# alessiomelone/Ternary-spGEMM

Measured on AMD Instinct MI355X. Metric: effective GFLOP/s + achieved HBM GB/s (% roofline), TCSC spGEMM M×K×N at s, higher is better.
Workload: dtype f32

## Files before the change

ternary-spgemm_amd/csrc/tsg_capi.cpp:

```cpp
#include <hip/hip_runtime.h>

#include <algorithm>
#include <cmath>
#include <cstdlib>
#include <cstdio>
#include <cstring>
#include <atomic>
#include <iterator>
#include <condition_variable>
#include <mutex>
#include <string>
#include <thread>
#include <vector>

#include "../../include/ternary_spgemm_test.h"
#include "tsg_internal.h"
#include "tsg_plan.h"

using tsg::CallPlan;
using tsg::JitShape;
using tsg::Kernel;

extern thread_local std::string g_tsg_host_err;

// ... 61 lines not shown
namespace {

struct DeviceGuard {
    int prev = -1;
    explicit DeviceGuard(int dev)
    {
        if (hipGetDevice(&prev) != hipSuccess) prev = -1;
        if (dev >= 0 && dev != prev) (void)hipSetDevice(dev);
    }
    ~DeviceGuard()
    {
        if (prev >= 0) (void)hipSetDevice(prev);
    }
};

int check_device(int dev)
{
    hipDeviceProp_t prop;
    if (hipGetDeviceProperties(&prop, dev) != hipSuccess)
        return fail(TSG_ERR_NODEV, "hipGetDeviceProperties failed for device " + std::to_string(dev));
    if (std::strncmp(prop.gcnArchName, "gfx950", 6) != 0)
        return fail(TSG_ERR_NODEV, std::string("device is ") + prop.gcnArchName +
                                       "; this library is built for gfx950 (MI355X) only");
    return TSG_OK;
}

struct XtDims {
    int Mp, Kp;
};
XtDims dims_for(int M, int K, int tile_m, int chunk)
{
    return {((std::max(M, 1) + tile_m - 1) / tile_m) * tile_m, std::max(1, (K + chunk - 1) / chunk) * chunk};
}

int ensure_work(tsg_tcsc *h, int M, int tile_m, int chunk, bool capturing)
{
    const XtDims d = dims_for(M, h->plan.K, tile_m, chunk);
    const size_t need = (size_t)d.Mp * d.Kp * sizeof(float);
// ... 295 lines not shown
    if (!direct) {
        rc = work_begin(h, p, c);
        if (rc) return rc;
        if (K == 0) {
            HIP_TRY(hipMemsetAsync(h->d_work, 0, (size_t)d.Mp * d.Kp * sizeof(float), c.s));
        } else if ((r64 ? tsg::launch_transpose_quads(c.dX, h->d_work, c.M, K, d.Mp, d.Kp, jv.piece_rows, c.s, p.chunk)
                        : tsg::launch_transpose_pairs(c.dX, h->d_work, c.M, K, d.Mp, d.Kp, c.s)) != 0) {
            return fail(TSG_ERR_HIP, std::string("transpose launch: ") + hipGetErrorString(hipGetLastError()));
        }
    }
    int slot;
    rc = timing_begin(h, c.capturing, c.s, slot);
    if (rc) return rc;
    if (tsg::launch_tcsc_jit(jv.mod, direct ? c.dX : h->d_work, d.Mp, jv.d_wcode, c.db, c.dalpha, c.dY, c.M, N, jv.Npad,
                             jv.nch, c.prelu ? 1 : 0, h->d_status, jv.nw * jv.waves, waves, p.gn, p.gm, p.tmask, c.s,
                             p.tile_m, direct ? K : 0, lastadj, p.xtouch, p.tnear) != 0)
        return fail(TSG_ERR_HIP, std::string("tcsc launch: ") + hipGetErrorString(hipGetLastError()));
    rc = timing_end(h, slot, c.s);
    if (rc || direct) return rc;
    return work_end(h, c);
}

int run_dev(tsg_tcsc *h, const float *dX, const float *db, const float *dalpha, float *dY, int M,
            int N, int K, hipStream_t s, bool prelu)
{
    if (!h) return fail(TSG_ERR_ARG, "null handle");
    if (N != h->plan.N || K != h->plan.K)
        return fail(TSG_ERR_ARG, "shape mismatch: handle has K=" + std::to_string(h->plan.K) + " N=" +
                                     std::to_string(h->plan.N) + ", call has K=" + std::to_string(K) +
                                     " N=" + std::to_string(N));
    if (M < 0) return fail(TSG_ERR_ARG, "M < 0");
// ... 219 lines not shown
{
    if (!out) return fail(TSG_ERR_ARG, "null out");
    *out = nullptr;
    if (B < 0) return fail(TSG_ERR_ARG, "negative block size");
    const std::string ke = tsg::knob_check();
    if (!ke.empty()) return fail(TSG_ERR_ARG, ke);
    std::string e = tsg::validate_tcsc(csp, csn, rip, rin, K, N, B);
    if (!e.empty()) return fail(TSG_ERR_ARG, std::string(B ? "malformed BlockedTCSC: " : "malformed TCSC: ") + e);
    if (B && (tsg::kJitXRegs - tsg::kJitNW) / tsg::kJitSlotRegs < 2)
        return fail(TSG_ERR_ARG, "BlockedTCSC: this jit kernel geometry has no registers for the block sums");
    const int64_t slots = (B ? (int64_t)(K / B) : 1) * N;
    int ndev = 0;
    if (hipGetDeviceCount(&ndev) != hipSuccess || ndev == 0) return fail(TSG_ERR_NODEV, "no HIP device");
    if (device < 0) HIP_TRY(hipGetDevice(&device));
    if (device >= ndev) return fail(TSG_ERR_ARG, "device index out of range");
    int rc = check_device(device);
    if (rc) return rc;

    tsg_tcsc *h = new tsg_tcsc();
    h->plan.K = K;
    h->plan.N = N;
    h->plan.B = B;
    h->device = device;
    {
        DeviceGuard g0(device);
        if (hipStreamCreateWithFlags(&h->stream, hipStreamNonBlocking) != hipSuccess) {
            delete h;
            return fail(TSG_ERR_HIP, "hipStreamCreate of the handle's stream failed");
        }
    }
    h->nnz_pos = csp[slots];
    h->nnz_neg = csn[slots];
    h->plan.nnz = h->nnz_pos + h->nnz_neg;
    h->csp.assign(csp, csp + slots + 1);
// ... 336 lines not shown
    *gn = p.gn;
    *gm = p.gm;
    *tmask = p.tmask;
    return TSG_OK;
}

extern "C" int tsg_call_xtouch(int K, int N, int64_t nnz, int M)
{
    if (K < 0 || N <= 0 || nnz < 0 || nnz > (int64_t)K * N || M <= 0) {
        g_tsg_host_err = "tsg_call_xtouch: bad arguments";
        return TSG_ERR_ARG;
    }
    return tsg::plan_call(plain_input(K, N, nnz), M).xtouch;
}

extern "C" const char *tcsc_hip_call_kernel(const tsg_tcsc *h, int M)
{
    if (!h) return "";
    std::lock_guard<std::mutex> lk(h->mu);
    switch (tsg::plan_call(h->plan, M).kernel) {
    case Kernel::kEllPc: return "tsg_tcsc_ell_pc_kernel";
    case Kernel::kEll: return "tsg_tcsc_ell_kernel";
    case Kernel::kJit64: return "tsg_jit64_kernel";
    case Kernel::kJit128: return "tsg_jit_kernel";
    case Kernel::kRx: break;
    }
    return "tsg_tcsc_rx_kernel";
}

extern "C" int64_t tcsc_hip_call_image_bytes(tsg_tcsc *h, int M)
// ... 107 lines not shown
```

ternary-spgemm_amd/csrc/tsg_internal.h:

```cpp
#pragma once

#include <cstddef>
#include <cstdint>
#include <string>
#include <vector>

namespace tsg {

constexpr int kLanes = 64;

#ifndef TSG_RX_WAVES
#define TSG_RX_WAVES 8
#endif
#ifndef TSG_RX_CHUNK
#define TSG_RX_CHUNK 64
#endif
#ifndef TSG_RX_ROWS
#define TSG_RX_ROWS 24
#endif
constexpr int kRxTileM = 256;
constexpr int kRxWaves = TSG_RX_WAVES;
constexpr int kRxNW = 32;
constexpr int kRxTileCols = kRxWaves * kRxNW;
constexpr int kRxChunk = TSG_RX_CHUNK;
// ... 68 lines not shown
                    const int32_t *rin, int K, int N, int B, JitImage &img, int nw = kJitNW,
                    int waves = kJitWaves, bool far = false, bool rows64 = false, bool half = false);

struct JitModule {
    void *module = nullptr;
    void *function = nullptr;
    void *probe = nullptr;
    std::string load(const std::vector<uint32_t> &code, int nw = kJitNW, int waves = kJitWaves,
                     bool rows64 = false, bool half = false, bool pair = false);
    void unload();
};
int launch_tcsc_jit(const JitModule &jm, const float *XT, int Mp, const uint32_t *wcode,
                    const float *b, const float *alpha, float *Y, int M, int N, int Npad, int nch,
                    int prelu, uint32_t *status, int tile_cols, int waves, int gn, int gm, int tmask,
                    void *stream, int tile_m = kJitTileM, int xrow = 0, int lastadj = 0, int xtouch = 0,
                    int tnear = 0);
int launch_jit_probe(const JitModule &jm, uint32_t *status, void *stream);

constexpr int kEllVariants = 5;
constexpr int kEllTileM[kEllVariants] = {1, 4, 8, 16, 32};
constexpr int kEllMaxC[kEllVariants] = {40956, 10236, 5116, 2556, 1276};
struct EllImage {
    int C = 0, nch = 0, steps = 0, nslices = 0;
    int xb = 0;
    int zr = 1;
    std::vector<uint32_t> ent;
    std::vector<uint32_t> tab;
};
constexpr int ell_copy_offset(int C, int MT) { return ((C + 1) * MT + 63) / 64 * 64 + 32; }
__host__ __device__ constexpr int ell_lds_floats(int C, int MT, int xb, int zr = 1)
{
// ... 35 lines not shown
```

ternary-spgemm_amd/csrc/tsg_jit.cpp:

```cpp
#include <hip/hip_runtime.h>

#include <dlfcn.h>
#include <elf.h>

#include <algorithm>
#include <cmath>
#include <cstdio>
#include <cstdlib>
#include <cstring>
#include <fstream>
#include <iterator>

#include "tsg_internal.h"
#include "tsg_jit_map.h"
#include "../../include/ternary_spgemm_test.h"

namespace tsg {

namespace {

struct Emit {
    std::vector<uint32_t> &c;
    bool pad8 = true;
    void align8()
// ... 788 lines not shown
    function = nullptr;
    probe = nullptr;
}

int launch_jit_probe(const JitModule &jm, uint32_t *status, void *stream)
{
    void *params[] = {(void *)&status};
    const hipError_t e =
        hipModuleLaunchKernel((hipFunction_t)jm.probe, 1, 1, 1, 64, 1, 1, 0, (hipStream_t)stream, params, nullptr);
    return e == hipSuccess ? 0 : -1;
}

int launch_tcsc_jit(const JitModule &jm, const float *XT, int Mp, const uint32_t *wcode, const float *b,
                    const float *alpha, float *Y, int M, int N, int Npad, int nch, int prelu,
                    uint32_t *status, int tile_cols, int waves, int gn, int gm, int tmask, void *stream,
                    int tile_m, int xrow, int lastadj, int xtouch, int tnear)
{
    int mtiles = Mp / tile_m, ntiles = Npad / tile_cols;
    void *params[] = {(void *)&XT, (void *)&Mp, (void *)&wcode, (void *)&b, (void *)&alpha, (void *)&Y,
                      (void *)&M, (void *)&N, (void *)&nch, (void *)&mtiles, (void *)&ntiles, (void *)&prelu,
                      (void *)&status, (void *)&gn, (void *)&gm, (void *)&tmask, (void *)&xrow, (void *)&lastadj,
                      (void *)&xtouch, (void *)&tnear};
    hipError_t e = hipModuleLaunchKernel((hipFunction_t)jm.function, (unsigned)(mtiles * ntiles), 1, 1,
                                         (unsigned)waves * 64u, 1, 1, 0, (hipStream_t)stream, params, nullptr);
    return e == hipSuccess ? 0 : -1;
}

}

extern thread_local std::string g_tsg_host_err;

extern "C" int tsg_jit_codegen_wv(const int32_t *csp, const int32_t *csn, const int32_t *rip, const int32_t *rin,
                                  int K, int N, int B, int width, int waves, uint32_t *code, int64_t code_cap,
                                  int64_t *code_len, uint32_t *wcode, int64_t wcode_cap, int64_t *wcode_len)
{
    if (!tsg::jit_waves_ok(width, waves)) {
        g_tsg_host_err = "tsg_jit_codegen: unsupported waves per workgroup " + std::to_string(waves) +
                         " for width " + std::to_string(width) + " (8; 4 for widths 32, 16, 8)";
// ... 158 lines not shown
```

ternary-spgemm_amd/csrc/tsg_jit_kernel.hip:

```cpp
#include <hip/hip_runtime.h>

#include <cstdint>

#include "tsg_jit_map.h"

namespace {

#ifndef TSG_JIT_NW
#define TSG_JIT_NW 64
#endif
#ifndef TSG_JIT_WAVES
#define TSG_JIT_WAVES 8
#endif
#ifndef TSG_JIT_ROWS64
#define TSG_JIT_ROWS64 0
#endif
#ifndef TSG_JIT_HALF
#define TSG_JIT_HALF 0
#endif
#ifndef TSG_JIT_PAIR
#define TSG_JIT_PAIR 0
#endif
constexpr int kJWaves = TSG_JIT_WAVES;
constexpr int kJNW = TSG_JIT_NW;
constexpr bool kJRows64 = TSG_JIT_ROWS64 != 0;
constexpr bool kJHalf = TSG_JIT_HALF != 0;
constexpr bool kJPair = TSG_JIT_PAIR != 0;
static_assert(!kJHalf || (kJRows64 && TSG_JIT_WAVES == 4), "the half ring is a 4-wave 64-row image");
static_assert(!kJPair || (kJRows64 && TSG_JIT_WAVES == 4 && !kJHalf), "wave pairs run the 4-wave 64-row image");
static_assert(kJNW == 64 || kJNW == 32 || kJNW == 16 || kJNW == 8 || (kJRows64 && kJNW == 128), "stream width");
static_assert(kJWaves == 8 || (kJWaves == 4 && kJNW < 64), "waves per workgroup");
constexpr int kJTileM = kJRows64 ? 64 : 128;
constexpr int kJRowsPerLane = kJTileM / 64;
constexpr int kJTileCols = kJWaves * kJNW;
constexpr int kJThreads = (kJPair ? 2 : 1) * kJWaves * 64;
constexpr int kJRing = 3;
constexpr int kJChunk = kJRows64 ? (kJHalf ? 96 : 192) : 96;
// ... 76 lines not shown

    uint64_t base;
    asm volatile("s_getpc_b64 s[92:93]\n\t"
                 "s_add_u32 s92, s92, 0x7a5e1234\n\t"
                 "s_addc_u32 s93, s93, 0"
                 : "={s[92:93]}"(base)
                 :
                 : "scc");
    const uint32_t *hdr = reinterpret_cast<const uint32_t *>(base);
    if (hdr[0] != kJMagic0 || hdr[1] != kJMagic1 || ((hdr[7] >> 8) & 0xffu) != kJFormat ||
        ((hdr[7] & kJHalfFlag) != 0) != kJHalf) {
        if (blockIdx.x == 0 && tid == 0) status[0] = 1u;
        return;
    }

    int nt, mt;
    tsg_jit_tile(blockIdx.x, mtiles, ntiles, gn, gm, nt, mt);
    const int m0 = mt * kJTileM;
    const int stream = wave;
    const int ncol0 = nt * kJTileCols + stream * kJNW;
    const uint64_t cp = base + __builtin_amdgcn_readfirstlane(wcode[(size_t)nt * kJWaves + stream]);
    const uint32_t pr_rows = (hdr[7] & kJR16Flag) ? 16u : 8u;
    const bool rowlay = kJRows64 && !kJHalf && (__builtin_amdgcn_readfirstlane(hdr[7]) & kJRowFlag) != 0;
    const uint32_t lb0 = rowlay   ? (uint32_t)lane * 752u
                         : kJRows64 ? ((uint32_t)lane / pr_rows) * 1024u + ((uint32_t)lane % pr_rows) * 16u
                                    : (uint32_t)lane * 16u;
    const uint32_t lb1 = lb0 + kJBufBytes, lb2 = lb0 + 2 * kJBufBytes;
    const uint32_t m0k = (hdr[7] & kJM0kFlag) ? 1u : 0u;
    uint32_t off[kJPieces];
    const bool direct = kJRows64 && xrow > 0;
    const uint32_t xrow_b = (uint32_t)xrow * 4u;
#pragma unroll
    for (int i = 0; i < kJPieces; i++) {
        const uint32_t pr = (uint32_t)(wave * kJPieces + i);
        uint32_t o;
        if (!kJRows64) {
            o = (pr * ((uint32_t)Mp / 2u) + (uint32_t)m0 / 2u + (uint32_t)lane) * 16u;
        } else if (rowlay) {
            const uint32_t slot = min(pr * 64u + (uint32_t)lane, 64u * 47u - 1u);
            const uint32_t row = slot / 47u, quad = slot % 47u;
            o = direct ? (uint32_t)min(m0 + (int)row, M - 1) * xrow_b + quad * 16u + 3072u
                       : ((uint32_t)mt * 47u + pr) * 1024u + (uint32_t)lane * 16u;
        } else if (direct) {
            const uint32_t rgs = 64u / pr_rows;
            const uint32_t row = (uint32_t)min(m0 + (int)((pr % rgs) * pr_rows + (uint32_t)lane % pr_rows), M - 1);
            o = row * xrow_b + ((pr / rgs) * rgs + (uint32_t)lane / pr_rows) * 16u + 3072u;
        } else {
            o = ((uint32_t)mt * (uint32_t)kJUnits + pr) * 1024u + (uint32_t)lane * 16u;
        }
        off[i] = o - m0k * (uint32_t)(i & 3) * 1024u;
    }
    const uint64_t xbase = (uint64_t)(uintptr_t)XT - (direct ? 3072u : 0u);
    const uint32_t wb = (uint32_t)(wave * kJPieces) * 1024u;
    const uint32_t l128 = (mt & tmask) == 0 ? (uint32_t)lane * 128u : 0u;
    const uint32_t l128x = xtouch ? l128 : 0u;
    const uint64_t tbase = base - (tnear ? 8192u : 0u);
    const uint32_t chunk_rows = rowlay ? 188u : (uint32_t)kJChunk;
    const uint32_t stride = direct ? chunk_rows * 4u : chunk_rows * (uint32_t)Mp * 4u;
    const uint32_t adj = direct ? (uint32_t)lastadj : 0u;

#if TSG_JIT_PAIR
    const uint64_t emask = rhalf ? 0xffffffff00000000ull : 0x00000000ffffffffull;
    uint64_t esave;
#define TSG_JIT_EXEC_IN "s_mov_b64 %[es], exec\n\ts_mov_b64 exec, %[em]\n\t"
#define TSG_JIT_EXEC_OUT "\n\ts_mov_b64 exec, %[es]"
#define TSG_JIT_EXEC_OPS , [es] "=&s"(esave)
#define TSG_JIT_EXEC_INS , [em] "s"(emask)
#else
#define TSG_JIT_EXEC_IN ""
#define TSG_JIT_EXEC_OUT ""
#define TSG_JIT_EXEC_OPS
#define TSG_JIT_EXEC_INS
#endif
#define TSG_JIT_CALL(...)                                                                           \
    asm volatile(TSG_JIT_EXEC_IN                                                                    \
                 "s_getpc_b64 s[94:95]\n"                                                           \
                 ".Ljr%=:\n\t"                                                                      \
                 "s_add_u32 s94, s94, (.Ljb%= - .Ljr%=)\n\t"                                        \
// ... 5 lines not shown
                   "{s83}"(wb), "{s87}"(adj),                                                          \
                   TSG_JIT_IN TSG_JIT_EXEC_INS                                                      \
                 : TSG_JIT_CLOBBERS)
#if TSG_JIT_ROWS64
#if TSG_JIT_WAVES == 8 || TSG_JIT_HALF
#define TSG_JIT_A0 "v[116:147]"
#define TSG_JIT_A1 "v[148:179]"
#define TSG_JIT_A16 "v[116:131]"
#define TSG_JIT_A8 "v[116:123]"
#else
#define TSG_JIT_A0 "v[122:153]"
#define TSG_JIT_A16 "v[122:137]"
#define TSG_JIT_A8 "v[122:129]"
#endif
#if TSG_JIT_NW == 128
    F32x32 a0 = {}, a1 = {}, a2 = {}, a3 = {};
    TSG_JIT_CALL("+{v[116:147]}"(a0), "+{v[148:179]}"(a1), "+{v[180:211]}"(a2), "+{v[212:243]}"(a3));
    auto acc_of = [&](int c, int) { return c < 32 ? a0[c] : c < 64 ? a1[c - 32] : c < 96 ? a2[c - 64] : a3[c - 96]; };
#elif TSG_JIT_NW == 64
    F32x32 a0 = {}, a1 = {};
    TSG_JIT_CALL("+{" TSG_JIT_A0 "}"(a0), "+{" TSG_JIT_A1 "}"(a1));
    auto acc_of = [&](int c, int) { return c < 32 ? a0[c] : a1[c - 32]; };
#elif TSG_JIT_NW == 32
    F32x32 a0 = {};
    TSG_JIT_CALL("+{" TSG_JIT_A0 "}"(a0));
    auto acc_of = [&](int c, int) { return a0[c]; };
#elif TSG_JIT_NW == 16
    F32x16 a0 = {};
    TSG_JIT_CALL("+{" TSG_JIT_A16 "}"(a0));
    auto acc_of = [&](int c, int) { return a0[c]; };
#else
    F32x8 a0 = {};
    TSG_JIT_CALL("+{" TSG_JIT_A8 "}"(a0));
    auto acc_of = [&](int c, int) { return a0[c]; };
#endif
#elif TSG_JIT_WAVES == 8 && TSG_JIT_NW == 64
    F32x32 a0 = {}, a1 = {}, a2 = {}, a3 = {};
    TSG_JIT_CALL("+{v[116:147]}"(a0), "+{v[148:179]}"(a1), "+{v[180:211]}"(a2), "+{v[212:243]}"(a3));
    auto acc_of = [&](int c, int r) {
        return c < 16 ? a0[2 * (c & 15) + r] : c < 32 ? a1[2 * (c & 15) + r]
             : c < 48 ? a2[2 * (c & 15) + r] : a3[2 * (c & 15) + r];
    };
#elif TSG_JIT_WAVES == 8 && TSG_JIT_NW == 32
    F32x32 a0 = {}, a1 = {};
    TSG_JIT_CALL("+{v[116:147]}"(a0), "+{v[148:179]}"(a1));
    auto acc_of = [&](int c, int r) { return c < 16 ? a0[2 * (c & 15) + r] : a1[2 * (c & 15) + r]; };
#elif TSG_JIT_WAVES == 8 && TSG_JIT_NW == 16
    F32x32 a0 = {};
    TSG_JIT_CALL("+{v[116:147]}"(a0));
    auto acc_of = [&](int c, int r) { return a0[2 * c + r]; };
#elif TSG_JIT_WAVES == 8
    F32x16 a0 = {};
    TSG_JIT_CALL("+{v[116:131]}"(a0));
    auto acc_of = [&](int c, int r) { return a0[2 * c + r]; };
#elif TSG_JIT_NW == 32
    F32x32 a0 = {}, a1 = {};
    TSG_JIT_CALL("+{v[122:153]}"(a0), "+{v[154:185]}"(a1));
    auto acc_of = [&](int c, int r) { return c < 16 ? a0[2 * (c & 15) + r] : a1[2 * (c & 15) + r]; };
#elif TSG_JIT_NW == 16
    F32x32 a0 = {};
    TSG_JIT_CALL("+{v[122:153]}"(a0));
    auto acc_of = [&](int c, int r) { return a0[2 * c + r]; };
#else
    F32x16 a0 = {};
    TSG_JIT_CALL("+{v[122:137]}"(a0));
    auto acc_of = [&](int c, int r) { return a0[2 * c + r]; };
#endif
#undef TSG_JIT_CALL

    if (ncol0 >= N) return;
    if (kJPair && (lane >> 5) != rhalf) return;
#pragma unroll
    for (int r = 0; r < kJRowsPerLane; r++) {
        const int m = m0 + kJRowsPerLane * lane + r;
        if (m >= M) continue;
        float *yrow = Y + (size_t)m * N + ncol0;
        float v[kJNW];
#pragma unroll
        for (int c = 0; c < kJNW; c++) {
            const int n = ncol0 + c < N ? ncol0 + c : N - 1;
            const float acc = acc_of(c, r);
            float y = acc + b[n];
            if (prelu) y = (y > 0) ? y : alpha[n] * y;
            v[c] = y;
        }
        if (ncol0 + kJNW <= N && (((uintptr_t)yrow & 15) == 0)) {
#pragma unroll
            for (int c = 0; c < kJNW; c += 4)
                *reinterpret_cast<float4 *>(yrow + c) = make_float4(v[c], v[c + 1], v[c + 2], v[c + 3]);
        } else {
#pragma unroll
            for (int c = 0; c < kJNW; c++)
                if (ncol0 + c < N) yrow[c] = v[c];
        }
    }
}
```

ternary-spgemm_amd/csrc/tsg_knobs.cpp:

```cpp
#include <cerrno>
#include <cmath>
#include <cstdlib>
#include <cstring>
#include <string>
#include <vector>

#include "tsg_internal.h"
#include "../../include/ternary_spgemm_test.h"

namespace tsg {

namespace {

std::vector<std::string> fields(const char *v)
{
    std::vector<std::string> out(1);
    for (const char *p = v; *p; p++) {
        if (*p == ',') out.emplace_back();
        else out.back() += *p;
    }
    return out;
}

bool parse_i64(const std::string &s, int64_t lo, int64_t hi, int base = 10)
// ... 81 lines not shown
    {"TSG_JIT_NOALIGN", "0 | 1", [](const char *v) { return one_of(v, {"0", "1"}); }},
    {"TSG_JIT_GN", "1..1024", [](const char *v) { return int_in(v, 1, 1024); }},
    {"TSG_JIT_GM", "1..1024", [](const char *v) { return int_in(v, 1, 1024); }},
    {"TSG_JIT_TMASK", "0..255", [](const char *v) { return int_in(v, 0, 255); }},
    {"TSG_JIT_DMA", "spread[0..1],m0k[0|1][,lag[1|2]]", dma_ok},
    {"TSG_JIT_CP", "dma,touch (hex, bits of 0x2030000)", cp_ok},
    {"TSG_JIT_TOUCH", "first,count (8-KiB units, first >= 1, count <= 4)", touch_ok},
    {"TSG_JIT_READS", "G,RA (G >= 1, G + RA <= 24)", reads_ok},
    {"TSG_JIT_TGROUP", "0 | 1 | 2", [](const char *v) { return one_of(v, {"0", "1", "2"}); }},
    {"TSG_JIT_XTOUCH", "0 | 1", [](const char *v) { return one_of(v, {"0", "1"}); }},
    {"TSG_JIT_TNEAR", "0 | 1", [](const char *v) { return one_of(v, {"0", "1"}); }},
    {"TSG_JIT_TGAP", "0..65536 (bytes)", [](const char *v) { return int_in(v, 0, 65536); }},
    {"TSG_JIT_TROLL", "0..8 (rolling code touches, 8-KiB windows ahead)", [](const char *v) { return int_in(v, 0, 8); }},
    {"TSG_JIT_MIX", "reads,dma (0|1 each)",
     [](const char *v) { return one_of(v, {"0,0", "0,1", "1,0", "1,1"}); }},
    {"TSG_JIT_DIR", "a directory", [](const char *v) { return *v != '\0'; }},
    {"TSG_ELL_PC", "0 | 1", [](const char *v) { return one_of(v, {"0", "1"}); }},
    {"TSG_ELL_MAXM", "0..1024", [](const char *v) { return int_in(v, 0, 1024); }},
    {"TSG_ELL_PC_MAXMN", "0..2^40", [](const char *v) { return int_in(v, 0, 1ll << 40); }},
    {"TSG_ELL_VARIANT", "0..4", [](const char *v) { return int_in(v, 0, kEllVariants - 1); }},
    {"TSG_ELL_LA", "1 | 2", [](const char *v) { return one_of(v, {"1", "2"}); }},
    {"TSG_ELL_LG", "2 | 4 | 8 | 16", [](const char *v) { return one_of(v, {"2", "4", "8", "16"}); }},
    {"TSG_ELL_PC_E", "16 | 32 | 64", [](const char *v) { return one_of(v, {"16", "32", "64"}); }},
    {"TSG_ELL_COPIES", "1 | 2", [](const char *v) { return one_of(v, {"1", "2"}); }},
    {"TSG_ELL_WPG", "4 | 8 | 16", [](const char *v) { return one_of(v, {"4", "8", "16"}); }},
    {"TSG_ELL_SCHED", "0 | 1", [](const char *v) { return one_of(v, {"0", "1"}); }},
#ifdef TSG_DIAG
    {"TSG_JIT_DIAG", "nobar,nodma,notouch,nolgkm,noreads,novm,samecode,samewave,pairwave,simdpair,balance4,balance1,anti4", diag_ok},
#endif
};
// ... 50 lines not shown
```

ternary-spgemm_amd/csrc/tsg_plan.cpp:

```cpp
#include "tsg_plan.h"

#include <algorithm>
#include <cstdlib>

#include "tsg_internal.h"

namespace tsg {

namespace {

constexpr int kEllAutoMaxM = 32;
constexpr int kEllAutoMaxMChunked = 16;
constexpr int64_t kEllPcRowsMaxMN = 32768;
constexpr int kEllStarvedMaxM = 1024;
constexpr int kEllSmallWMaxM = 128;
constexpr double kEllSmallWWork = 420e6;
constexpr int kRows64AutoMaxM = 512;
constexpr double kRows64FullRound = 0.9;
constexpr int64_t kJitFullWgs = 230;
constexpr int64_t kJitOneRoundWgs = 256;
constexpr double kFarXtBytes = 768.0 * 1024 * 1024;
constexpr double kFarCodeBytes = 160.0 * 1024 * 1024;
constexpr double kFarKeepXtBytes = 1536.0 * 1024 * 1024;
constexpr double kXDirectMinAddsPerRow = 32.0;
// ... 263 lines not shown
    if (!sh.r64) return false;
    if (piece_rows < 0)
        piece_rows = sh.half ? (jit64_piece_rows() ? jit64_piece_rows() : 16) : jit64_piece_rows();
    const char *e = knob_value("TSG_JIT_XDIRECT");
    const bool on = e ? e[0] == '1' : x_direct_auto(in, sh.nw, piece_rows);
    return on && x_direct_shape_ok(in.K, piece_rows) && x_aligned && x_direct_offsets_ok(M, in.K);
}

bool may_fall_back(const PlanInput &in, const JitShape &sh)
{
    const bool is_default = !sh.r64 && !sh.far && sh.nw == kJitNW && sh.waves == kJitWaves;
    return !is_default && !in.tile_rows && !in.jit_force && in.far_mode != 2 &&
           !knob_value("TSG_JIT_ROWS64_MAXM") && !knob_value("TSG_JIT_NW");
}

CallPlan plan_call(const PlanInput &in, int M)
{
    CallPlan p;
    p.xtouch = pick_xtouch(in, M) ? 1 : 0;
    p.ell = pick_ell_variant(in, M);
    if (p.ell >= 0) {
        p.kernel = use_ell_pc(in, p.ell) ? Kernel::kEllPc : Kernel::kEll;
        return p;
    }
    if (!in.jit) {
        p.kernel = Kernel::kRx;
        p.tile_m = kRxTileM;
        p.chunk = kRxChunk;
        return p;
    }
// ... 25 lines not shown
```

ternary-spgemm_amd/csrc/tsg_plan.h:

```cpp
#pragma once

#include <cstdint>

namespace tsg {

struct JitShape {
    int nw, waves;
    bool far = false;
    bool r64 = false;
    bool half = false;
};

int width_index(int nw);
int shape_index(int nw, int waves, bool far = false);
int shape_index(const JitShape &sh);
int variant_bit(const JitShape &sh);

struct PlanInput {
    int K = 0, N = 0;
    int B = 0;
    int64_t nnz = 0;
    bool jit = true;
    int tile_rows = 0;
    int jit_force = 0;
    int far_mode = 0;
    int small_m = 0;
    uint32_t bad_variants = 0;
    int jit_nch = 0;
};

enum class Kernel { kRx, kJit128, kJit64, kEll, kEllPc };

struct CallPlan {
    Kernel kernel = Kernel::kRx;
    int ell = -1;
    JitShape shape{0, 0};
    int tile_m = 0, chunk = 0;
    int gn = 0, gm = 0, tmask = 0;
    int tnear = 0;
    int xtouch = 0;
    bool is_ell() const { return kernel == Kernel::kEll || kernel == Kernel::kEllPc; }
    bool is_jit() const { return kernel == Kernel::kJit128 || kernel == Kernel::kJit64; }
};

CallPlan plan_call(const PlanInput &in, int M);

bool x_direct(const PlanInput &in, const JitShape &sh, int piece_rows, bool x_aligned, int M);

bool may_fall_back(const PlanInput &in, const JitShape &sh);

constexpr int kEllTile8 = 2;
constexpr int kEllMidM = 32;

constexpr int kHostChunksMax = 16;
int host_chunk_rows(const PlanInput &in, int host_chunks, int M);

}
```

ternary-spgemm_amd/tspgemm.py:

```python
from __future__ import annotations

import ctypes as C
import os
import subprocess
from typing import Callable, List, Optional, Tuple

import numpy as np

PKG_DIR = os.path.dirname(os.path.abspath(__file__))
LIB_PATH = os.environ.get("TSG_LIB") or os.path.join(PKG_DIR, "lib", "libternary_spgemm.so")

TSG_OK = 0
_ERRNAMES = {1: "TSG_ERR_ARG", 2: "TSG_ERR_HIP", 3: "TSG_ERR_NOMEM", 4: "TSG_ERR_NODEV",
             5: "TSG_ERR_RANGE"}

EXPORTED_SYMBOLS = (
    "tcsc_hip_create", "tcsc_hip_create_dense", "tcsc_hip_destroy", "tcsc_hip_gemm",
    "tcsc_hip_gemm_dev", "tcsc_hip_gemm_prelu", "tcsc_hip_gemm_prelu_dev", "tcsc_hip_reserve",
    "tcsc_hip_info", "tcsc_hip_to_dense", "tcsc_hip_set_timing", "tcsc_hip_kernel_time",
    "tcsc_hip_last_error", "tcsc_hip_device_count", "tsg_tcsc_slice", "tsg_tcsc_validate",
    "tsg_gen_tcsc", "tsg_gen_x", "tcsc_hip_create_csc_packed", "tsg_tcsc_to_csc_packed",
    "tsg_csc_packed_to_tcsc", "tsg_jit_codegen", "tcsc_hip_kernel_name", "tcsc_hip_encode_dense_dev",
    "tcsc_hip_create_blocked", "tsg_jit_codegen_blocked", "tsg_blocked_tcsc_validate",
    "tcsc_hip_jit_width", "tcsc_hip_set_jit_width", "tcsc_hip_jit_waves", "tsg_jit_codegen_w", "tsg_jit_codegen_wv",
    "tcsc_hip_set_small_m", "tcsc_hip_call_kernel", "tsg_ell_build", "tsg_jit_tile_map",
    "tcsc_hip_set_host_chunks", "tcsc_hip_host_chunk_rows", "tcsc_hip_call_image_bytes",
    "tcsc_hip_host_register", "tcsc_hip_host_unregister", "tcsc_hip_set_far", "tcsc_hip_call_far",
    "tsg_jit_codegen_far", "tsg_call_plan", "tsg_call_xtouch", "tsg_knob_check", "tcsc_hip_set_tile_rows", "tcsc_hip_call_tile_rows",
    "tsg_jit_codegen64", "tsg_jit_codegen64h", "tcsc_hip_call_launches",
)


class TSGError(RuntimeError):
    def __init__(self, code: int, where: str, msg: str):
        super().__init__(f"{where}: {_ERRNAMES.get(code, code)}: {msg}")
        self.code = code


class tsg_info(C.Structure):
    _fields_ = [("K", C.c_int32), ("N", C.c_int32), ("device", C.c_int32),
                ("abi_version", C.c_int32), ("nnz_pos", C.c_int64), ("nnz_neg", C.c_int64),
                ("tcsc_bytes", C.c_int64), ("image_bytes", C.c_int64), ("work_bytes", C.c_int64),
                ("chunk_rows", C.c_int32), ("tile_rows", C.c_int32), ("tile_cols", C.c_int32),
# ... 60 lines not shown
    L.tsg_jit_codegen_w.argtypes = [vp, vp, vp, vp, C.c_int, C.c_int, C.c_int, C.c_int, vp, C.c_int64,
                                    C.POINTER(C.c_int64), vp, C.c_int64, C.POINTER(C.c_int64)]
    L.tsg_jit_codegen_wv.argtypes = [vp, vp, vp, vp, C.c_int, C.c_int, C.c_int, C.c_int, C.c_int, vp, C.c_int64,
                                     C.POINTER(C.c_int64), vp, C.c_int64, C.POINTER(C.c_int64)]
    L.tcsc_hip_set_small_m.argtypes = [H, C.c_int]
    L.tcsc_hip_set_far.argtypes = [H, C.c_int]
    L.tcsc_hip_set_tile_rows.argtypes = [H, C.c_int]
    L.tcsc_hip_call_tile_rows.argtypes = [H, C.c_int]
    L.tcsc_hip_call_launches.argtypes = [H, C.c_void_p, C.c_int]
    L.tsg_jit_codegen64.argtypes = [vp, vp, vp, vp, C.c_int, C.c_int, C.c_int, C.c_int, vp, C.c_int64,
                                    C.POINTER(C.c_int64), vp, C.c_int64, C.POINTER(C.c_int64)]
    L.tsg_jit_codegen64h.argtypes = [vp, vp, vp, vp, C.c_int, C.c_int, C.c_int, vp, C.c_int64,
                                     C.POINTER(C.c_int64), vp, C.c_int64, C.POINTER(C.c_int64)]
    L.tsg_call_plan.argtypes = [C.c_int, C.c_int, C.c_int64, C.c_int] + [C.POINTER(C.c_int)] * 7
    L.tsg_call_xtouch.argtypes = [C.c_int, C.c_int, C.c_int64, C.c_int]
    L.tcsc_hip_call_far.argtypes = [H, C.c_int]
    L.tsg_jit_codegen_far.argtypes = [vp, vp, vp, vp, C.c_int, C.c_int, vp, C.c_int64,
                                      C.POINTER(C.c_int64), vp, C.c_int64, C.POINTER(C.c_int64)]
    L.tcsc_hip_set_host_chunks.argtypes = [H, C.c_int]
    L.tcsc_hip_host_chunk_rows.argtypes = [H, C.c_int]
    L.tcsc_hip_call_image_bytes.argtypes = [H, C.c_int]
    L.tcsc_hip_host_register.argtypes = [vp, C.c_size_t]
    L.tcsc_hip_host_unregister.argtypes = [vp]
    L.tcsc_hip_call_kernel.argtypes = [H, C.c_int]
    L.tcsc_hip_call_kernel.restype = C.c_char_p
    L.tsg_knob_check.argtypes = []
    L.tsg_knob_check.restype = C.c_char_p
    L.tsg_ell_build.argtypes = [vp, vp, vp, vp, C.c_int, C.c_int, C.c_int, C.c_int, C.c_int, vp, C.c_int64,
                                C.POINTER(C.c_int64), vp, C.c_int64, C.POINTER(C.c_int64), C.POINTER(C.c_int32),
                                C.POINTER(C.c_int32), C.POINTER(C.c_int32)]
# ... 145 lines not shown

def call_plan(K: int, N: int, nnz: int, M: int) -> dict:
    v = [C.c_int() for _ in range(7)]
    _check(lib().tsg_call_plan(K, N, nnz, M, *[C.byref(x) for x in v]), "tsg_call_plan")
    kernel, width, waves, far, gn, gm, tmask = (x.value for x in v)
    return {"kernel": ("tsg_jit_kernel", "tsg_tcsc_ell_kernel", "tsg_tcsc_ell_pc_kernel", "tsg_jit64_kernel")[kernel],
            "width": width, "waves": waves, "far": bool(far), "map": (gn, gm), "tmask": tmask}


def call_xtouch(K: int, N: int, nnz: int, M: int) -> bool:
    r = lib().tsg_call_xtouch(K, N, nnz, M)
    _check(min(r, 0), "tsg_call_xtouch")
    return bool(r)


def jit_tile_map(L: int, mtiles: int, ntiles: int, gn: int, gm: int):
    nt, mt = C.c_int(), C.c_int()
    _check(lib().tsg_jit_tile_map(L, mtiles, ntiles, gn, gm, C.byref(nt), C.byref(mt)), "tsg_jit_tile_map")
    return nt.value, mt.value


def ell_build(csp, csn, rip, rin, K: int, N: int, Cmax: int, MT: int, copies: int = 1, with_xb: bool = False):
    csp, csn, rip, rin = _i32(csp), _i32(csn), _i32(rip), _i32(rin)
    ne, nt, c, nch, xb = C.c_int64(), C.c_int64(), C.c_int32(), C.c_int32(), C.c_int32()
    L = lib()
    _check(L.tsg_ell_build(_ptr(csp), _ptr(csn), _ptr(rip), _ptr(rin), K, N, Cmax, MT, copies, None, 0, C.byref(ne),
                           None, 0, C.byref(nt), C.byref(c), C.byref(nch), C.byref(xb)), "tsg_ell_build")
    ent = np.empty(ne.value, np.uint32)
    tab = np.empty(nt.value, np.uint32)
    _check(L.tsg_ell_build(_ptr(csp), _ptr(csn), _ptr(rip), _ptr(rin), K, N, Cmax, MT, copies, _ptr(ent), ne.value,
# ... 248 lines not shown
    def set_small_m(self, mode: int) -> None:
        _check(lib().tcsc_hip_set_small_m(self._h, mode), "tcsc_hip_set_small_m")

    def set_host_chunks(self, chunks: int) -> None:
        _check(lib().tcsc_hip_set_host_chunks(self._h, chunks), "tcsc_hip_set_host_chunks")

    def host_chunk_rows(self, M: int) -> int:
        return int(lib().tcsc_hip_host_chunk_rows(self._h, M))

    def call_image_bytes(self, M: int) -> int:
        return int(lib().tcsc_hip_call_image_bytes(self._h, M))

    def call_kernel(self, M: int) -> str:
        return lib().tcsc_hip_call_kernel(self._h, M).decode()

    def set_far(self, mode: int) -> None:
        _check(lib().tcsc_hip_set_far(self._h, mode), "tcsc_hip_set_far")

    def set_tile_rows(self, rows: int) -> None:
        _check(lib().tcsc_hip_set_tile_rows(self._h, rows), "tcsc_hip_set_tile_rows")

    def call_tile_rows(self, M: int) -> int:
        return int(lib().tcsc_hip_call_tile_rows(self._h, M))

    def call_launches(self, X, M: int) -> int:
        ptr = X.data_ptr() if hasattr(X, "data_ptr") else int(X)
        return int(lib().tcsc_hip_call_launches(self._h, C.c_void_p(ptr), M))

    def call_far(self, M: int) -> bool:
        return bool(lib().tcsc_hip_call_far(self._h, M))
# ... 54 lines not shown
```

Baseline: 58380.

## Make rows64 JIT kernel persistent with grid sized to CU count

Wraps the rows64 JIT kernel body in a grid-stride loop over tiles. The launch grid is capped at the device's compute-unit count (rounded down to a multiple of 8) instead of one workgroup per tile, and a barrier separates consecutive tiles. The aim is to cut workgroup launch and dispatch overhead and the tail imbalance, at the cost of less latency hiding from oversubscription and an extra barrier per tile. Knobs allow disabling it or overriding the grid size.

```diff
diff --git a/ternary-spgemm_amd/csrc/tsg_capi.cpp b/ternary-spgemm_amd/csrc/tsg_capi.cpp
--- a/ternary-spgemm_amd/csrc/tsg_capi.cpp
+++ b/ternary-spgemm_amd/csrc/tsg_capi.cpp
@@ -99,7 +99,7 @@
     }
 };
 
-int check_device(int dev)
+int check_device(int dev, int &cus)
 {
     hipDeviceProp_t prop;
     if (hipGetDeviceProperties(&prop, dev) != hipSuccess)
@@ -107,6 +107,7 @@
     if (std::strncmp(prop.gcnArchName, "gfx950", 6) != 0)
         return fail(TSG_ERR_NODEV, std::string("device is ") + prop.gcnArchName +
                                        "; this library is built for gfx950 (MI355X) only");
+    cus = prop.multiProcessorCount;
     return TSG_OK;
 }
 
@@ -432,7 +433,8 @@
     if (rc) return rc;
     if (tsg::launch_tcsc_jit(jv.mod, direct ? c.dX : h->d_work, d.Mp, jv.d_wcode, c.db, c.dalpha, c.dY, c.M, N, jv.Npad,
                              jv.nch, c.prelu ? 1 : 0, h->d_status, jv.nw * jv.waves, waves, p.gn, p.gm, p.tmask, c.s,
-                             p.tile_m, direct ? K : 0, lastadj, p.xtouch, p.tnear) != 0)
+                             p.tile_m, direct ? K : 0, lastadj, p.xtouch, p.tnear,
+                             tsg::persist_grid(h->plan, p.shape, jv.pair, wgs)) != 0)
         return fail(TSG_ERR_HIP, std::string("tcsc launch: ") + hipGetErrorString(hipGetLastError()));
     rc = timing_end(h, slot, c.s);
     if (rc || direct) return rc;
@@ -682,10 +684,12 @@
     if (hipGetDeviceCount(&ndev) != hipSuccess || ndev == 0) return fail(TSG_ERR_NODEV, "no HIP device");
     if (device < 0) HIP_TRY(hipGetDevice(&device));
     if (device >= ndev) return fail(TSG_ERR_ARG, "device index out of range");
-    int rc = check_device(device);
+    int cus = 0;
+    int rc = check_device(device, cus);
     if (rc) return rc;
 
     tsg_tcsc *h = new tsg_tcsc();
+    h->plan.slots = cus;
     h->plan.K = K;
     h->plan.N = N;
     h->plan.B = B;
@@ -1052,6 +1056,44 @@
     return tsg::plan_call(plain_input(K, N, nnz), M).xtouch;
 }
 
+extern "C" int tsg_call_grid(int K, int N, int64_t nnz, int M, int slots, int *workgroups, int *tiles)
+{
+    if (K < 0 || N <= 0 || nnz < 0 || nnz > (int64_t)K * N || M <= 0 || slots < 0 || !workgroups || !tiles) {
+        g_tsg_host_err = "tsg_call_grid: bad arguments";
+        return TSG_ERR_ARG;
+    }
+    tsg::PlanInput in = plain_input(K, N, nnz);
+    in.slots = slots;
+    const CallPlan p = tsg::plan_call(in, M);
+    *workgroups = *tiles = 0;
+    if (!p.is_jit()) return TSG_OK;
+    const int cols = p.shape.nw * p.shape.waves;
+    *tiles = ((M + p.tile_m - 1) / p.tile_m) * ((N + cols - 1) / cols);
+    const char *pv = tsg::knob_value("TSG_JIT_PAIR");
+    const bool pair = p.shape.r64 && p.shape.waves == 4 && !p.shape.half && pv && pv[0] == '1';
+    *workgroups = tsg::persist_grid(in, p.shape, pair, *tiles);
+    return TSG_OK;
+}
+
+extern "C" int tcsc_hip_call_grid(tsg_tcsc *h, int M, int *workgroups, int *tiles)
+{
+    if (!h || M <= 0 || !workgroups || !tiles) {
+        g_tsg_host_err = "tcsc_hip_call_grid: bad arguments";
+        return TSG_ERR_ARG;
+    }
+    std::lock_guard<std::mutex> lk(h->mu);
+    const CallPlan p = tsg::plan_call(h->plan, M);
+    *workgroups = *tiles = 0;
+    if (!p.is_jit()) return TSG_OK;
+    const int cols = p.shape.nw * p.shape.waves;
+    *tiles = ((M + p.tile_m - 1) / p.tile_m) * ((h->plan.N + cols - 1) / cols);
+    const tsg_tcsc::JitVariant &v = variant_of(h, p.shape);
+    const char *pv = tsg::knob_value("TSG_JIT_PAIR");
+    const bool pair = v.mod.function ? v.pair : p.shape.r64 && p.shape.waves == 4 && !p.shape.half && pv && pv[0] == '1';
+    *workgroups = tsg::persist_grid(h->plan, p.shape, pair, *tiles);
+    return TSG_OK;
+}
+
 extern "C" const char *tcsc_hip_call_kernel(const tsg_tcsc *h, int M)
 {
     if (!h) return "";
diff --git a/ternary-spgemm_amd/csrc/tsg_internal.h b/ternary-spgemm_amd/csrc/tsg_internal.h
--- a/ternary-spgemm_amd/csrc/tsg_internal.h
+++ b/ternary-spgemm_amd/csrc/tsg_internal.h
@@ -106,7 +106,7 @@
                     const float *b, const float *alpha, float *Y, int M, int N, int Npad, int nch,
                     int prelu, uint32_t *status, int tile_cols, int waves, int gn, int gm, int tmask,
                     void *stream, int tile_m = kJitTileM, int xrow = 0, int lastadj = 0, int xtouch = 0,
-                    int tnear = 0);
+                    int tnear = 0, int grid = 0);
 int launch_jit_probe(const JitModule &jm, uint32_t *status, void *stream);
 
 constexpr int kEllVariants = 5;
diff --git a/ternary-spgemm_amd/csrc/tsg_jit.cpp b/ternary-spgemm_amd/csrc/tsg_jit.cpp
--- a/ternary-spgemm_amd/csrc/tsg_jit.cpp
+++ b/ternary-spgemm_amd/csrc/tsg_jit.cpp
@@ -826,14 +826,15 @@
 int launch_tcsc_jit(const JitModule &jm, const float *XT, int Mp, const uint32_t *wcode, const float *b,
                     const float *alpha, float *Y, int M, int N, int Npad, int nch, int prelu,
                     uint32_t *status, int tile_cols, int waves, int gn, int gm, int tmask, void *stream,
-                    int tile_m, int xrow, int lastadj, int xtouch, int tnear)
+                    int tile_m, int xrow, int lastadj, int xtouch, int tnear, int grid)
 {
     int mtiles = Mp / tile_m, ntiles = Npad / tile_cols;
+    if (grid <= 0 || grid > mtiles * ntiles) grid = mtiles * ntiles;
     void *params[] = {(void *)&XT, (void *)&Mp, (void *)&wcode, (void *)&b, (void *)&alpha, (void *)&Y,
                       (void *)&M, (void *)&N, (void *)&nch, (void *)&mtiles, (void *)&ntiles, (void *)&prelu,
                       (void *)&status, (void *)&gn, (void *)&gm, (void *)&tmask, (void *)&xrow, (void *)&lastadj,
                       (void *)&xtouch, (void *)&tnear};
-    hipError_t e = hipModuleLaunchKernel((hipFunction_t)jm.function, (unsigned)(mtiles * ntiles), 1, 1,
+    hipError_t e = hipModuleLaunchKernel((hipFunction_t)jm.function, (unsigned)grid, 1, 1,
                                          (unsigned)waves * 64u, 1, 1, 0, (hipStream_t)stream, params, nullptr);
     return e == hipSuccess ? 0 : -1;
 }
diff --git a/ternary-spgemm_amd/csrc/tsg_jit_kernel.hip b/ternary-spgemm_amd/csrc/tsg_jit_kernel.hip
--- a/ternary-spgemm_amd/csrc/tsg_jit_kernel.hip
+++ b/ternary-spgemm_amd/csrc/tsg_jit_kernel.hip
@@ -21,6 +21,7 @@
 #ifndef TSG_JIT_PAIR
 #define TSG_JIT_PAIR 0
 #endif
+#define TSG_JIT_PERSIST (TSG_JIT_ROWS64 && !TSG_JIT_HALF && !TSG_JIT_PAIR)
 constexpr int kJWaves = TSG_JIT_WAVES;
 constexpr int kJNW = TSG_JIT_NW;
 constexpr bool kJRows64 = TSG_JIT_ROWS64 != 0;
@@ -127,54 +128,67 @@
         return;
     }
 
-    int nt, mt;
-    tsg_jit_tile(blockIdx.x, mtiles, ntiles, gn, gm, nt, mt);
-    const int m0 = mt * kJTileM;
-    const int stream = wave;
-    const int ncol0 = nt * kJTileCols + stream * kJNW;
-    const uint64_t cp = base + __builtin_amdgcn_readfirstlane(wcode[(size_t)nt * kJWaves + stream]);
-    const uint32_t pr_rows = (hdr[7] & kJR16Flag) ? 16u : 8u;
-    const bool rowlay = kJRows64 && !kJHalf && (__builtin_amdgcn_readfirstlane(hdr[7]) & kJRowFlag) != 0;
+    const uint32_t hflags = __builtin_amdgcn_readfirstlane(hdr[7]);
+    const uint32_t pr_rows = (hflags & kJR16Flag) ? 16u : 8u;
+    const bool rowlay = kJRows64 && !kJHalf && (hflags & kJRowFlag) != 0;
     const uint32_t lb0 = rowlay   ? (uint32_t)lane * 752u
                          : kJRows64 ? ((uint32_t)lane / pr_rows) * 1024u + ((uint32_t)lane % pr_rows) * 16u
                                     : (uint32_t)lane * 16u;
     const uint32_t lb1 = lb0 + kJBufBytes, lb2 = lb0 + 2 * kJBufBytes;
-    const uint32_t m0k = (hdr[7] & kJM0kFlag) ? 1u : 0u;
-    uint32_t off[kJPieces];
-    const bool direct = kJRows64 && xrow > 0;
-    const uint32_t xrow_b = (uint32_t)xrow * 4u;
-#pragma unroll
-    for (int i = 0; i < kJPieces; i++) {
-        const uint32_t pr = (uint32_t)(wave * kJPieces + i);
-        uint32_t o;
-        if (!kJRows64) {
-            o = (pr * ((uint32_t)Mp / 2u) + (uint32_t)m0 / 2u + (uint32_t)lane) * 16u;
-        } else if (rowlay) {
-            const uint32_t slot = min(pr * 64u + (uint32_t)lane, 64u * 47u - 1u);
-            const uint32_t row = slot / 47u, quad = slot % 47u;
-            o = direct ? (uint32_t)min(m0 + (int)row, M - 1) * xrow_b + quad * 16u + 3072u
-                       : ((uint32_t)mt * 47u + pr) * 1024u + (uint32_t)lane * 16u;
-        } else if (direct) {
-            const uint32_t rgs = 64u / pr_rows;
-            const uint32_t row = (uint32_t)min(m0 + (int)((pr % rgs) * pr_rows + (uint32_t)lane % pr_rows), M - 1);
-            o = row * xrow_b + ((pr / rgs) * rgs + (uint32_t)lane / pr_rows) * 16u + 3072u;
-        } else {
-            o = ((uint32_t)mt * (uint32_t)kJUnits + pr) * 1024u + (uint32_t)lane * 16u;
+    const uint32_t m0k = (hflags & kJM0kFlag) ? 1u : 0u;
+    const int stream = wave;
+
+    int L = blockIdx.x;
+#if TSG_JIT_PERSIST
+    const int tiles = mtiles * ntiles, lstep = gridDim.x;
+    const int lane_wg = lane;
+    for (;;) {
+        int lane_tile = lane_wg;
+        asm volatile("" : "+v"(lane_tile));
+        const int lane = lane_tile;
+#else
+    {
+#endif
+        int nt, mt;
+        tsg_jit_tile(L, mtiles, ntiles, gn, gm, nt, mt);
+        const int m0 = mt * kJTileM;
+        const int ncol0 = nt * kJTileCols + stream * kJNW;
+        const uint64_t cp = base + __builtin_amdgcn_readfirstlane(wcode[(size_t)nt * kJWaves + stream]);
+        uint32_t off[kJPieces];
+        const bool direct = kJRows64 && xrow > 0;
+        const uint32_t xrow_b = (uint32_t)xrow * 4u;
+#pragma unroll
+        for (int i = 0; i < kJPieces; i++) {
+            const uint32_t pr = (uint32_t)(wave * kJPieces + i);
+            uint32_t o;
+            if (!kJRows64) {
+                o = (pr * ((uint32_t)Mp / 2u) + (uint32_t)m0 / 2u + (uint32_t)lane) * 16u;
+            } else if (rowlay) {
+                const uint32_t slot = min(pr * 64u + (uint32_t)lane, 64u * 47u - 1u);
+                const uint32_t row = slot / 47u, quad = slot % 47u;
+                o = direct ? (uint32_t)min(m0 + (int)row, M - 1) * xrow_b + quad * 16u + 3072u
+                           : ((uint32_t)mt * 47u + pr) * 1024u + (uint32_t)lane * 16u;
+            } else if (direct) {
+                const uint32_t rgs = 64u / pr_rows;
+                const uint32_t row = (uint32_t)min(m0 + (int)((pr % rgs) * pr_rows + (uint32_t)lane % pr_rows), M - 1);
+                o = row * xrow_b + ((pr / rgs) * rgs + (uint32_t)lane / pr_rows) * 16u + 3072u;
+            } else {
+                o = ((uint32_t)mt * (uint32_t)kJUnits + pr) * 1024u + (uint32_t)lane * 16u;
+            }
+            off[i] = o - m0k * (uint32_t)(i & 3) * 1024u;
         }
-        off[i] = o - m0k * (uint32_t)(i & 3) * 1024u;
-    }
-    const uint64_t xbase = (uint64_t)(uintptr_t)XT - (direct ? 3072u : 0u);
-    const uint32_t wb = (uint32_t)(wave * kJPieces) * 1024u;
-    const uint32_t l128 = (mt & tmask) == 0 ? (uint32_t)lane * 128u : 0u;
-    const uint32_t l128x = xtouch ? l128 : 0u;
-    const uint64_t tbase = base - (tnear ? 8192u : 0u);
-    const uint32_t chunk_rows = rowlay ? 188u : (uint32_t)kJChunk;
-    const uint32_t stride = direct ? chunk_rows * 4u : chunk_rows * (uint32_t)Mp * 4u;
-    const uint32_t adj = direct ? (uint32_t)lastadj : 0u;
+        const uint64_t xbase = (uint64_t)(uintptr_t)XT - (direct ? 3072u : 0u);
+        const uint32_t wb = (uint32_t)(wave * kJPieces) * 1024u;
+        const uint32_t l128 = (mt & tmask) == 0 ? (uint32_t)lane * 128u : 0u;
+        const uint32_t l128x = xtouch ? l128 : 0u;
+        const uint64_t tbase = base - (tnear ? 8192u : 0u);
+        const uint32_t chunk_rows = rowlay ? 188u : (uint32_t)kJChunk;
+        const uint32_t stride = direct ? chunk_rows * 4u : chunk_rows * (uint32_t)Mp * 4u;
+        const uint32_t adj = direct ? (uint32_t)lastadj : 0u;
 
 #if TSG_JIT_PAIR
-    const uint64_t emask = rhalf ? 0xffffffff00000000ull : 0x00000000ffffffffull;
-    uint64_t esave;
+        const uint64_t emask = rhalf ? 0xffffffff00000000ull : 0x00000000ffffffffull;
+        uint64_t esave;
 #define TSG_JIT_EXEC_IN "s_mov_b64 %[es], exec\n\ts_mov_b64 exec, %[em]\n\t"
 #define TSG_JIT_EXEC_OUT "\n\ts_mov_b64 exec, %[es]"
 #define TSG_JIT_EXEC_OPS , [es] "=&s"(esave)
@@ -210,84 +224,89 @@
 #define TSG_JIT_A8 "v[122:129]"
 #endif
 #if TSG_JIT_NW == 128
-    F32x32 a0 = {}, a1 = {}, a2 = {}, a3 = {};
-    TSG_JIT_CALL("+{v[116:147]}"(a0), "+{v[148:179]}"(a1), "+{v[180:211]}"(a2), "+{v[212:243]}"(a3));
-    auto acc_of = [&](int c, int) { return c < 32 ? a0[c] : c < 64 ? a1[c - 32] : c < 96 ? a2[c - 64] : a3[c - 96]; };
+        F32x32 a0 = {}, a1 = {}, a2 = {}, a3 = {};
+        TSG_JIT_CALL("+{v[116:147]}"(a0), "+{v[148:179]}"(a1), "+{v[180:211]}"(a2), "+{v[212:243]}"(a3));
+        auto acc_of = [&](int c, int) { return c < 32 ? a0[c] : c < 64 ? a1[c - 32] : c < 96 ? a2[c - 64] : a3[c - 96]; };
 #elif TSG_JIT_NW == 64
-    F32x32 a0 = {}, a1 = {};
-    TSG_JIT_CALL("+{" TSG_JIT_A0 "}"(a0), "+{" TSG_JIT_A1 "}"(a1));
-    auto acc_of = [&](int c, int) { return c < 32 ? a0[c] : a1[c - 32]; };
+        F32x32 a0 = {}, a1 = {};
+        TSG_JIT_CALL("+{" TSG_JIT_A0 "}"(a0), "+{" TSG_JIT_A1 "}"(a1));
+        auto acc_of = [&](int c, int) { return c < 32 ? a0[c] : a1[c - 32]; };
 #elif TSG_JIT_NW == 32
-    F32x32 a0 = {};
-    TSG_JIT_CALL("+{" TSG_JIT_A0 "}"(a0));
-    auto acc_of = [&](int c, int) { return a0[c]; };
+        F32x32 a0 = {};
+        TSG_JIT_CALL("+{" TSG_JIT_A0 "}"(a0));
+        auto acc_of = [&](int c, int) { return a0[c]; };
 #elif TSG_JIT_NW == 16
-    F32x16 a0 = {};
-    TSG_JIT_CALL("+{" TSG_JIT_A16 "}"(a0));
-    auto acc_of = [&](int c, int) { return a0[c]; };
-#else
-    F32x8 a0 = {};
-    TSG_JIT_CALL("+{" TSG_JIT_A8 "}"(a0));
-    auto acc_of = [&](int c, int) { return a0[c]; };
+        F32x16 a0 = {};
+        TSG_JIT_CALL("+{" TSG_JIT_A16 "}"(a0));
+        auto acc_of = [&](int c, int) { return a0[c]; };
+#else
+        F32x8 a0 = {};
+        TSG_JIT_CALL("+{" TSG_JIT_A8 "}"(a0));
+        auto acc_of = [&](int c, int) { return a0[c]; };
 #endif
 #elif TSG_JIT_WAVES == 8 && TSG_JIT_NW == 64
-    F32x32 a0 = {}, a1 = {}, a2 = {}, a3 = {};
-    TSG_JIT_CALL("+{v[116:147]}"(a0), "+{v[148:179]}"(a1), "+{v[180:211]}"(a2), "+{v[212:243]}"(a3));
-    auto acc_of = [&](int c, int r) {
-        return c < 16 ? a0[2 * (c & 15) + r] : c < 32 ? a1[2 * (c & 15) + r]
-             : c < 48 ? a2[2 * (c & 15) + r] : a3[2 * (c & 15) + r];
-    };
+        F32x32 a0 = {}, a1 = {}, a2 = {}, a3 = {};
+        TSG_JIT_CALL("+{v[116:147]}"(a0), "+{v[148:179]}"(a1), "+{v[180:211]}"(a2), "+{v[212:243]}"(a3));
+        auto acc_of = [&](int c, int r) {
+            return c < 16 ? a0[2 * (c & 15) + r] : c < 32 ? a1[2 * (c & 15) + r]
+                 : c < 48 ? a2[2 * (c & 15) + r] : a3[2 * (c & 15) + r];
+        };
 #elif TSG_JIT_WAVES == 8 && TSG_JIT_NW == 32
-    F32x32 a0 = {}, a1 = {};
-    TSG_JIT_CALL("+{v[116:147]}"(a0), "+{v[148:179]}"(a1));
-    auto acc_of = [&](int c, int r) { return c < 16 ? a0[2 * (c & 15) + r] : a1[2 * (c & 15) + r]; };
+        F32x32 a0 = {}, a1 = {};
+        TSG_JIT_CALL("+{v[116:147]}"(a0), "+{v[148:179]}"(a1));
+        auto acc_of = [&](int c, int r) { return c < 16 ? a0[2 * (c & 15) + r] : a1[2 * (c & 15) + r]; };
 #elif TSG_JIT_WAVES == 8 && TSG_JIT_NW == 16
-    F32x32 a0 = {};
-    TSG_JIT_CALL("+{v[116:147]}"(a0));
-    auto acc_of = [&](int c, int r) { return a0[2 * c + r]; };
+        F32x32 a0 = {};
+        TSG_JIT_CALL("+{v[116:147]}"(a0));
+        auto acc_of = [&](int c, int r) { return a0[2 * c + r]; };
 #elif TSG_JIT_WAVES == 8
-    F32x16 a0 = {};
-    TSG_JIT_CALL("+{v[116:131]}"(a0));
-    auto acc_of = [&](int c, int r) { return a0[2 * c + r]; };
+        F32x16 a0 = {};
+        TSG_JIT_CALL("+{v[116:131]}"(a0));
+        auto acc_of = [&](int c, int r) { return a0[2 * c + r]; };
 #elif TSG_JIT_NW == 32
-    F32x32 a0 = {}, a1 = {};
-    TSG_JIT_CALL("+{v[122:153]}"(a0), "+{v[154:185]}"(a1));
-    auto acc_of = [&](int c, int r) { return c < 16 ? a0[2 * (c & 15) + r] : a1[2 * (c & 15) + r]; };
+        F32x32 a0 = {}, a1 = {};
+        TSG_JIT_CALL("+{v[122:153]}"(a0), "+{v[154:185]}"(a1));
+        auto acc_of = [&](int c, int r) { return c < 16 ? a0[2 * (c & 15) + r] : a1[2 * (c & 15) + r]; };
 #elif TSG_JIT_NW == 16
-    F32x32 a0 = {};
-    TSG_JIT_CALL("+{v[122:153]}"(a0));
-    auto acc_of = [&](int c, int r) { return a0[2 * c + r]; };
-#else
-    F32x16 a0 = {};
-    TSG_JIT_CALL("+{v[122:137]}"(a0));
-    auto acc_of = [&](int c, int r) { return a0[2 * c + r]; };
+        F32x32 a0 = {};
+        TSG_JIT_CALL("+{v[122:153]}"(a0));
+        auto acc_of = [&](int c, int r) { return a0[2 * c + r]; };
+#else
+        F32x16 a0 = {};
+        TSG_JIT_CALL("+{v[122:137]}"(a0));
+        auto acc_of = [&](int c, int r) { return a0[2 * c + r]; };
 #endif
 #undef TSG_JIT_CALL
 
-    if (ncol0 >= N) return;
-    if (kJPair && (lane >> 5) != rhalf) return;
-#pragma unroll
-    for (int r = 0; r < kJRowsPerLane; r++) {
-        const int m = m0 + kJRowsPerLane * lane + r;
-        if (m >= M) continue;
-        float *yrow = Y + (size_t)m * N + ncol0;
-        float v[kJNW];
-#pragma unroll
-        for (int c = 0; c < kJNW; c++) {
-            const int n = ncol0 + c < N ? ncol0 + c : N - 1;
-            const float acc = acc_of(c, r);
-            float y = acc + b[n];
-            if (prelu) y = (y > 0) ? y : alpha[n] * y;
-            v[c] = y;
+        const bool stores = ncol0 < N && !(kJPair && (lane >> 5) != rhalf);
+#pragma unroll
+        for (int r = 0; r < kJRowsPerLane; r++) {
+            const int m = m0 + kJRowsPerLane * lane + r;
+            if (!stores || m >= M) continue;
+            float *yrow = Y + (size_t)m * N + ncol0;
+            float v[kJNW];
+#pragma unroll
+            for (int c = 0; c < kJNW; c++) {
+                const int n = ncol0 + c < N ? ncol0 + c : N - 1;
+                const float acc = acc_of(c, r);
+                float y = acc + b[n];
+                if (prelu) y = (y > 0) ? y : alpha[n] * y;
+                v[c] = y;
+            }
+            if (ncol0 + kJNW <= N && (((uintptr_t)yrow & 15) == 0)) {
+#pragma unroll
+                for (int c = 0; c < kJNW; c += 4)
+                    *reinterpret_cast<float4 *>(yrow + c) = make_float4(v[c], v[c + 1], v[c + 2], v[c + 3]);
+            } else {
+#pragma unroll
+                for (int c = 0; c < kJNW; c++)
+                    if (ncol0 + c < N) yrow[c] = v[c];
+            }
         }
-        if (ncol0 + kJNW <= N && (((uintptr_t)yrow & 15) == 0)) {
-#pragma unroll
-            for (int c = 0; c < kJNW; c += 4)
-                *reinterpret_cast<float4 *>(yrow + c) = make_float4(v[c], v[c + 1], v[c + 2], v[c + 3]);
-        } else {
-#pragma unroll
-            for (int c = 0; c < kJNW; c++)
-                if (ncol0 + c < N) yrow[c] = v[c];
-        }
+#if TSG_JIT_PERSIST
+        L += lstep;
+        if (L >= tiles) break;
+        asm volatile("s_barrier" ::: "memory");
+#endif
     }
 }
diff --git a/ternary-spgemm_amd/csrc/tsg_knobs.cpp b/ternary-spgemm_amd/csrc/tsg_knobs.cpp
--- a/ternary-spgemm_amd/csrc/tsg_knobs.cpp
+++ b/ternary-spgemm_amd/csrc/tsg_knobs.cpp
@@ -119,6 +119,8 @@
     {"TSG_JIT_TROLL", "0..8 (rolling code touches, 8-KiB windows ahead)", [](const char *v) { return int_in(v, 0, 8); }},
     {"TSG_JIT_MIX", "reads,dma (0|1 each)",
      [](const char *v) { return one_of(v, {"0,0", "0,1", "1,0", "1,1"}); }},
+    {"TSG_JIT_PERSIST", "0 | 1", [](const char *v) { return one_of(v, {"0", "1"}); }},
+    {"TSG_JIT_GRID", "1..65536 (workgroups)", [](const char *v) { return int_in(v, 1, 65536); }},
     {"TSG_JIT_DIR", "a directory", [](const char *v) { return *v != '\0'; }},
     {"TSG_ELL_PC", "0 | 1", [](const char *v) { return one_of(v, {"0", "1"}); }},
     {"TSG_ELL_MAXM", "0..1024", [](const char *v) { return int_in(v, 0, 1024); }},
diff --git a/ternary-spgemm_amd/csrc/tsg_plan.cpp b/ternary-spgemm_amd/csrc/tsg_plan.cpp
--- a/ternary-spgemm_amd/csrc/tsg_plan.cpp
+++ b/ternary-spgemm_amd/csrc/tsg_plan.cpp
@@ -301,6 +301,17 @@
            !knob_value("TSG_JIT_ROWS64_MAXM") && !knob_value("TSG_JIT_NW");
 }
 
+int persist_grid(const PlanInput &in, const JitShape &sh, bool pair, int64_t tiles)
+{
+    const int t = (int)tiles;
+    if (!sh.r64 || sh.half || pair) return t;
+    const char *pv = knob_value("TSG_JIT_PERSIST");
+    if (pv && pv[0] == '0') return t;
+    int grid = in.slots / 8 * 8;
+    if (const char *gv = knob_value("TSG_JIT_GRID")) grid = grid > 0 ? std::min(grid, atoi(gv)) : atoi(gv);
+    return grid > 0 ? std::min(t, grid) : t;
+}
+
 CallPlan plan_call(const PlanInput &in, int M)
 {
     CallPlan p;
diff --git a/ternary-spgemm_amd/csrc/tsg_plan.h b/ternary-spgemm_amd/csrc/tsg_plan.h
--- a/ternary-spgemm_amd/csrc/tsg_plan.h
+++ b/ternary-spgemm_amd/csrc/tsg_plan.h
@@ -27,6 +27,7 @@
     int small_m = 0;
     uint32_t bad_variants = 0;
     int jit_nch = 0;
+    int slots = 0;
 };
 
 enum class Kernel { kRx, kJit128, kJit64, kEll, kEllPc };
@@ -47,6 +48,8 @@
 
 bool x_direct(const PlanInput &in, const JitShape &sh, int piece_rows, bool x_aligned, int M);
 
+int persist_grid(const PlanInput &in, const JitShape &sh, bool pair, int64_t tiles);
+
 bool may_fall_back(const PlanInput &in, const JitShape &sh);
 
 constexpr int kEllTile8 = 2;
diff --git a/ternary-spgemm_amd/tspgemm.py b/ternary-spgemm_amd/tspgemm.py
--- a/ternary-spgemm_amd/tspgemm.py
+++ b/ternary-spgemm_amd/tspgemm.py
@@ -26,7 +26,7 @@
     "tcsc_hip_set_small_m", "tcsc_hip_call_kernel", "tsg_ell_build", "tsg_jit_tile_map",
     "tcsc_hip_set_host_chunks", "tcsc_hip_host_chunk_rows", "tcsc_hip_call_image_bytes",
     "tcsc_hip_host_register", "tcsc_hip_host_unregister", "tcsc_hip_set_far", "tcsc_hip_call_far",
-    "tsg_jit_codegen_far", "tsg_call_plan", "tsg_call_xtouch", "tsg_knob_check", "tcsc_hip_set_tile_rows", "tcsc_hip_call_tile_rows",
+    "tsg_jit_codegen_far", "tsg_call_plan", "tsg_call_xtouch", "tsg_call_grid", "tcsc_hip_call_grid", "tsg_knob_check", "tcsc_hip_set_tile_rows", "tcsc_hip_call_tile_rows",
     "tsg_jit_codegen64", "tsg_jit_codegen64h", "tcsc_hip_call_launches",
 )
 
@@ -117,6 +117,8 @@
                                      C.POINTER(C.c_int64), vp, C.c_int64, C.POINTER(C.c_int64)]
     L.tsg_call_plan.argtypes = [C.c_int, C.c_int, C.c_int64, C.c_int] + [C.POINTER(C.c_int)] * 7
     L.tsg_call_xtouch.argtypes = [C.c_int, C.c_int, C.c_int64, C.c_int]
+    L.tsg_call_grid.argtypes = [C.c_int, C.c_int, C.c_int64, C.c_int, C.c_int] + [C.POINTER(C.c_int)] * 2
+    L.tcsc_hip_call_grid.argtypes = [H, C.c_int] + [C.POINTER(C.c_int)] * 2
     L.tcsc_hip_call_far.argtypes = [H, C.c_int]
     L.tsg_jit_codegen_far.argtypes = [vp, vp, vp, vp, C.c_int, C.c_int, vp, C.c_int64,
                                       C.POINTER(C.c_int64), vp, C.c_int64, C.POINTER(C.c_int64)]
@@ -292,6 +294,12 @@
     return bool(r)
 
 
+def call_grid(K: int, N: int, nnz: int, M: int, slots: int = 256):
+    wg, t = C.c_int(), C.c_int()
+    _check(lib().tsg_call_grid(K, N, nnz, M, slots, C.byref(wg), C.byref(t)), "tsg_call_grid")
+    return wg.value, t.value
+
+
 def jit_tile_map(L: int, mtiles: int, ntiles: int, gn: int, gm: int):
     nt, mt = C.c_int(), C.c_int()
     _check(lib().tsg_jit_tile_map(L, mtiles, ntiles, gn, gm, C.byref(nt), C.byref(mt)), "tsg_jit_tile_map")
@@ -570,6 +578,11 @@
     def call_kernel(self, M: int) -> str:
         return lib().tcsc_hip_call_kernel(self._h, M).decode()
 
+    def call_grid(self, M: int):
+        wg, t = C.c_int(), C.c_int()
+        _check(lib().tcsc_hip_call_grid(self._h, M, C.byref(wg), C.byref(t)), "tcsc_hip_call_grid")
+        return wg.value, t.value
+
     def set_far(self, mode: int) -> None:
         _check(lib().tcsc_hip_set_far(self._h, mode), "tcsc_hip_set_far")
 
```

Result: no change. 58760 (median of 3 runs) (+0.7%).
